# simonhmartin/genomics_general

Measured on AMD Instinct MI355X. Metric: windows_per_sec, higher is better.
Workload: dtype u32 bit-planes / int32 counts / f64 statistics

## Files before the change

### genomics_general_amd/csrc/pg_abi.cpp

```cpp
#include "pg_ctx.h"

#include <sched.h>

#include <algorithm>
#include <chrono>
#include <cstdarg>
#include <cstdio>
#include <cstring>
#include <cstdlib>
#include <thread>

static thread_local char g_err[1024] = "";

int pg_fail(int code, const char *fmt, ...) {
    va_list ap;
    va_start(ap, fmt);
    vsnprintf(g_err, sizeof(g_err), fmt, ap);
    va_end(ap);
    return code;
}

static int usable_cpus() {
    int n = (int)std::thread::hardware_concurrency();
    if (n < 1) n = 1;
// ... 695 lines not shown
        int words = (int)((len + 31) / 32);
        acc += words;
        mw = std::max(mw, words);
        ml = std::max(ml, len);
    }
    h[3 * (size_t)n] = acc;
    if (total_words) *total_words = acc;
    if (max_words) *max_words = mw;
    if (max_len) *max_len = ml;
    rc0 = c->win.upload(h, 3 * (size_t)n + 1, c->stream);
    if (rc0 != PG_OK) return rc0;
    HIPCHK(hipEventRecord(c->win_ev, c->stream));
    return PG_OK;
}

template <class F>
static int pairwise_batches(pg_ctx *c, const int64_t *lo, const int64_t *hi, int n_win, bool dip, F consume) {
    const int N = c->n_hap, NP = c->NP;
    const int n_units = dip ? N / 2 : N;
    const int NPv = dip ? (NP % 64 ? (n_units + 31) / 32 * 32 : (n_units + 63) / 64 * 64) : NP;
    c->cN = n_units;
    c->cshift = dip ? 1 : 0;
    const int64_t mat_bytes = 4ll * N * N + 4ll * n_units * n_units;
    int grp = PG_GROUP;
    {
        int64_t blocks64 = 0;
        for (int w = 0; w < n_win; ++w) blocks64 += ((hi[w] - lo[w] + 31) / 32 + PG_GROUP - 1) / PG_GROUP;
        const int waves_per_block = (NP / 4 + 63) / 64;
        if (blocks64 * waves_per_block >= 32768) grp = PG_GROUP_MAX;
        else if (blocks64 * waves_per_block < 8192) grp = PG_GROUP / 2;
        if (const char *g = getenv("PG_GROUP_WORDS")) grp = std::min(PG_GROUP_MAX, std::max(8, atoi(g) / 4 * 4));
    }
    const int capg = c->xv_worst ? PG_XV_CAP(grp) : PG_XV_CAP_DEFAULT(grp);
    const int64_t word_bytes = ((int64_t)NP * 4 * PG_XV_PLANES * capg + grp - 1) / grp + (int64_t)NPv * 4;
    int64_t total_words_all = 0;
    for (int w = 0; w < n_win; ++w) total_words_all += ((hi[w] - lo[w] + 31) / 32 + grp - 1) / grp * grp;
    const bool multi = total_words_all * word_bytes + (int64_t)n_win * mat_bytes > c->scratch_limit;
    const bool two_streams = getenv("PG_OVERLAP") != nullptr;
    const int n_sub = two_streams && atoi(getenv("PG_OVERLAP")) >= 2 ? atoi(getenv("PG_OVERLAP")) : 8;
    const bool split = multi || two_streams;
    int64_t target_words = two_streams ? std::max<int64_t>(total_words_all / n_sub, 32768) : total_words_all;
    for (int k = 0; k < 2; ++k) {
        if (!c->slot[k].packed) HIPCHK(hipEventCreateWithFlags(&c->slot[k].packed, hipEventDisableTiming));
        if (!c->slot[k].consumed) HIPCHK(hipEventCreateWithFlags(&c->slot[k].consumed, hipEventDisableTiming));
        c->slot[k].used = false;
    }
    int w0 = 0, bi = 0;
    while (w0 < n_win) {
        int64_t words = 0;
        int w1 = w0;
        while (w1 < n_win) {
            int64_t wlen = ((hi[w1] - lo[w1] + 31) / 32 + grp - 1) / grp * grp;
            int64_t nbytes = (words + wlen) * word_bytes + (int64_t)(w1 - w0 + 1) * mat_bytes;
            if (w1 > w0 && (nbytes > (split ? c->scratch_limit / 2 : c->scratch_limit) || words + wlen > target_words)) break;
            words += wlen;
            ++w1;
            if (w1 - w0 >= 65535) break;
        }
        const int nb = w1 - w0;
        pg_ctx::Slot &sl = c->slot[bi & 1];
        int rc;
        const bool single = (w0 == 0 && w1 == n_win) || !two_streams;
        hipStream_t ps = single ? c->stream : c->stream2;
        if (sl.used) {
            HIPCHK(hipStreamWaitEvent(ps, sl.consumed, 0));
            HIPCHK(hipEventSynchronize(sl.packed));
        }
        int64_t ga_pre = 0;
        for (int k = 0; k < nb; ++k) ga_pre += ((hi[w0 + k] - lo[w0 + k] + 31) / 32 + grp - 1) / grp;
        const size_t n_nw = (size_t)nb + (pg_pack_needs_presence(NP) ? (size_t)ga_pre : 0);
        const size_t h_len = 4 * (size_t)nb + 2 + (n_nw + 1) / 2;
        if ((rc = sl.host.ensure(h_len)) != PG_OK) return rc;
        int64_t *h = sl.host.p;
        int64_t ga = 0, va = 0;
        int max_groups = 0;
        for (int k = 0; k < nb; ++k) {
            h[k] = lo[w0 + k];
            h[nb + k] = hi[w0 + k];
            const int64_t wds = (hi[w0 + k] - lo[w0 + k] + 31) / 32;
            h[2 * (size_t)nb + k] = ga;
            h[3 * (size_t)nb + 1 + k] = va;
            const int64_t groups = (wds + grp - 1) / grp;
            ga += groups;
            va += (wds + 3) / 4;
            max_groups = (int)std::max<int64_t>(max_groups, groups);
        }
        h[3 * (size_t)nb] = ga;
        h[4 * (size_t)nb + 1] = va;
        memset(h + 4 * (size_t)nb + 2, 0, ((n_nw + 1) / 2) * 8);
        if ((rc = sl.win.upload(h, h_len, ps)) != PG_OK) return rc;
        const int64_t *d_lo = sl.win.p, *d_hi = sl.win.p + nb, *d_goff = sl.win.p + 2 * (size_t)nb,
                      *d_vgoff = sl.win.p + 3 * (size_t)nb + 1;
        int32_t *d_nw = reinterpret_cast<int32_t *>(sl.win.p + 4 * (size_t)nb + 2);
        if ((rc = sl.Vp.ensure((size_t)(std::max<int64_t>(va, 1) + 4) * NPv * 4)) != PG_OK) return rc;
        if ((rc = sl.XV.ensure(((size_t)std::max<int64_t>(ga, 1) * capg + 4) * PG_XV_PLANES * NP)) != PG_OK) return rc;
        if ((rc = c->Cmat.ensure((size_t)nb * n_units * n_units)) != PG_OK) return rc;
        if ((rc = c->Dmat.ensure((size_t)nb * N * N)) != PG_OK) return rc;
        hipEvent_t e0, e1;
        const bool time_pack = (c->time_mask >> PG_K_PACK) & 1u;
        if (time_pack) {
            if ((rc = event_get(c, &e0)) != PG_OK) return rc;
            if ((rc = event_get(c, &e1)) != PG_OK) return rc;
            HIPCHK(hipEventRecord(e0, ps));
        }
        if (pg_pack_needs_presence(NP) && (rc = sl.pres.ensure((size_t)std::max<int64_t>(ga, 1) * grp * 4)) != PG_OK) return rc;
        pg_launch_pack2(ps, c->gt.p, c->RS, d_lo, d_hi, d_goff, d_vgoff, nb, max_groups, ga, sl.Vp.p, NPv, sl.XV.p, NP,
                        d_nw, dip ? 1 : 0, c->flag.p, sl.pres.p, capg, grp);
        if (time_pack) {
            HIPCHK(hipEventRecord(e1, ps));
            c->events[PG_K_PACK].push_back(std::make_pair(e0, e1));
            c->acc_launches[PG_K_PACK] += 1;
        }
        HIPCHK(hipEventRecord(sl.packed, ps));
        if (!single) HIPCHK(hipStreamWaitEvent(c->stream, sl.packed, 0));
        if ((rc = pg_time_begin(c, PG_K_PAIRWISE, &e0, &e1)) != PG_OK) return rc;
        const bool valu_pairs = getenv("PG_PAIR_VALU") != nullptr;
        if (valu_pairs && NP % 64) return pg_fail(PG_ERR_STATE, "PG_PAIR_VALU must be set before pg_set_samples (plane stride %d)", NP);
        if (!valu_pairs && pg_pair_big_fits(NPv, n_units)) {
            pg_launch_pairC_big(c->stream, sl.Vp.p, d_vgoff, nb, NPv, n_units, dip ? 1 : 0, va / nb, (int64_t)max_groups * grp * 32, c->Cmat.p);
        } else if (!valu_pairs && pg_pair_tile_fits(NPv)) {
            if (pg_launch_pairC_tile(c->stream, sl.Vp.p, d_vgoff, nb, NPv, n_units, dip ? 1 : 0, va / nb, (int64_t)max_groups * grp * 32, c->Cmat.p))
                return pg_fail(PG_ERR_HIP, "pair-kernel program upload failed");
        } else if (!valu_pairs) pg_launch_pairC_mfma(c->stream, sl.Vp.p, d_vgoff, nb, NPv, n_units, dip ? 1 : 0, va / nb, (int64_t)max_groups * grp * 32, c->Cmat.p);
        else if (dip) pg_launch_pairC(c->stream, sl.Vp.p, d_vgoff, nb, c->tasksC.p, c->n_tasksC, NPv, n_units, 1, va / nb, c->Cmat.p);
        else pg_launch_pairC(c->stream, sl.Vp.p, d_vgoff, nb, c->tasksCh.p, c->n_tasksCh, NPv, n_units, 0, va / nb, c->Cmat.p);
        if ((rc = pg_time_end(c, PG_K_PAIRWISE, e0, e1, 1)) != PG_OK) return rc;
        if ((rc = pg_time_begin(c, PG_K_PAIRD, &e0, &e1)) != PG_OK) return rc;
        if (!valu_pairs) pg_launch_pairD_mfma(c->stream, sl.XV.p, d_nw, d_goff, nb, NP, N, ga / nb * grp / 10, (int64_t)max_groups * capg * 32, c->Dmat.p, capg);
        else pg_launch_pairD(c->stream, sl.XV.p, d_nw, d_goff, nb, c->tasks2.p, c->n_tasks2, NP, N, ga / nb, c->Dmat.p, capg);
        if ((rc = pg_time_end(c, PG_K_PAIRD, e0, e1, 1)) != PG_OK) return rc;
        HIPCHK(hipGetLastError());
        c->cur_win_lo = d_lo;
        c->cur_win_hi = d_hi;
        if ((rc = consume(w0, nb)) != PG_OK) return rc;
        HIPCHK(hipEventRecord(sl.consumed, c->stream));
        sl.used = true;
        w0 = w1;
        ++bi;
    }
    for (int k = 0; k < 2; ++k)
        if (c->slot[k].used) HIPCHK(hipEventSynchronize(c->slot[k].packed));
    return PG_OK;
}

static int stream_wait(pg_ctx *c) {
    static const long spin_us = getenv("PG_SPIN_US") ? atol(getenv("PG_SPIN_US")) : 2000;
    if (spin_us > 0) {
        const auto t0 = std::chrono::steady_clock::now();
        for (;;) {
            hipError_t e = hipStreamQuery(c->stream);
            if (e == hipSuccess) return PG_OK;
            if (e != hipErrorNotReady) return pg_fail(PG_ERR_HIP, "hipStreamQuery: %s", hipGetErrorString(e));
            if (std::chrono::duration_cast<std::chrono::microseconds>(std::chrono::steady_clock::now() - t0).count() > spin_us) break;
        }
    }
    HIPCHK(hipStreamSynchronize(c->stream));
    return PG_OK;
}

static int flag_ready(pg_ctx *c) {
    if (c->flag.p) return PG_OK;
    int rc = c->flag.ensure(1);
    if (rc != PG_OK) return rc;
    HIPCHK(hipMemsetAsync(c->flag.p, 0, 4, c->stream));
    HIPCHK(hipStreamSynchronize(c->stream));
    return PG_OK;
}

static int note_flags(pg_ctx *c, int flag, bool *dip, bool *again) {
    *again = false;
    if (flag & PG_FLAG_XV_OVERFLOW) {
        if (c->xv_worst) return pg_fail(PG_ERR_STATE, "XV overflow with the worst-case reservation");
        c->xv_worst = true;
        for (int k = 0; k < 2; ++k) c->slot[k].XV.release();
        *again = true;
    }
    if (*dip && (flag & PG_FLAG_MISMATCH)) {
        *dip = false;
        *again = true;
    }
    return PG_OK;
}

template <class F>
static int pairwise_run(pg_ctx *c, const int64_t *lo, const int64_t *hi, int n_win, F consume) {
    bool dip = c->all_diploid && getenv("PG_NO_DIP") == nullptr;
    int rc;
    if ((rc = flag_ready(c)) != PG_OK) return rc;
    for (;;) {
        if ((rc = pairwise_batches(c, lo, hi, n_win, dip, consume)) != PG_OK) return rc;
        int32_t flag = 0;
        HIPCHK(hipMemcpyAsync(&flag, c->flag.p, 4, hipMemcpyDeviceToHost, c->stream));
        HIPCHK(hipMemsetAsync(c->flag.p, 0, 4, c->stream));
        HIPCHK(hipStreamSynchronize(c->stream));
        bool again;
        if ((rc = note_flags(c, flag, &dip, &again)) != PG_OK) return rc;
        if (!again) return PG_OK;
    }
}

extern "C" int pg_reserve_sites_tuned(pg_ctx *c, int64_t n_sites, int max_trials, double *probe_ms_out, int *n_trials_out,
                                      int *chosen_out) {
    if (!c) return pg_fail(PG_ERR_ARG, "null ctx");
// ... 801 lines not shown
```

### genomics_general_amd/csrc/pg_internal.h

```cpp
#pragma once
#include <hip/hip_runtime.h>
#include <stdint.h>
#include "../../include/popgen_hip.h"
#include "pg_nib.h"

#define PG_MAX_POPS 16
#define PG_SITES_PER_BLOCK 1024
#define PG_ABBA_SITES_PER_BLOCK 4096
#define PG_ABBA_NSUM 6
#define PG_FOURPOP_NSUM 14
#define PG_XV_PLANES 2

#define PG_GROUP 64
#define PG_GROUP_MAX 128
#define PG_XV_CAP(grp) (3 * (grp))
#define PG_XV_CAP_DEFAULT(grp) ((grp) + 1)
#define PG_NP_MAX_SITES 256
#define PG_FLAG_MISMATCH 1
#define PG_FLAG_XV_OVERFLOW 2

struct PgTask2 {
    int32_t row0, nsub, col0, lower;
};

struct PgSynthParams {
    uint64_t seed;
    int64_t first_site_index, scaf_len;
    int32_t n_dip, n_pops, var_thr, miss_thr;
};


void pg_launch_nib_pack(hipStream_t st, const int8_t *src, int S, int n_hap, int64_t n_rows, int8_t *gt, int RS);
void pg_launch_nib_expand(hipStream_t st, const int8_t *gt, int RS, int64_t n_rows, int8_t *dst, int S);
void pg_launch_synth(hipStream_t st, int8_t *gt, int RS, int n_hap, int64_t site0, int64_t n_sites,
                     const int32_t *slot_gen_hap, PgSynthParams p);

void pg_launch_popdist_fin(hipStream_t st, const int32_t *Cmat, const int32_t *Dmat, int N, int cN, int cshift, int n_win,
                           const int32_t *pop_start, int n_pops, int min_pair_sites, double *sum_out,
                           int64_t *cnt_out, int all_diploid, const int64_t *win_lo = nullptr, const int64_t *win_hi = nullptr,
                           long long skip_upto = -1);

void pg_launch_popdist_np(hipStream_t st, const int32_t *Cmat, const int32_t *Dmat, int N, int cN, int cshift, int n_win,
                          const int32_t *pop_start, int n_pops, const int32_t *ref_row, const int32_t *pop_rank,
                          const int32_t *task_tree, const int32_t *trees, int max_leaves, int max_side, int min_pair_sites,
                          double min_data, int do_pairs, double *sums, int64_t *cnts, double *out, const int64_t *win_lo,
                          const int64_t *win_hi, long long max_sites);

void pg_launch_indpair_fin(hipStream_t st, const int32_t *Cmat, const int32_t *Dmat, int N, int cN, int cshift, int n_win,
                           const int32_t *samp_start, const int32_t *samp_rank, int n_samp, int min_pair_sites, double *sum_out,
                           int64_t *cnt_out, int mean_mode);


void pg_launch_abba(hipStream_t st, const int8_t *gt, int RS, const int64_t *win_lo, const int64_t *win_hi,
                    int n_win, int max_chunks, const int32_t *pop_start, int p1, int p2, int p3, int p4,
                    double min_data, int sel, int nsum, double *part_sums, int64_t *part_used, double *sums_out,
                    int64_t *used_out, uint32_t *flags, int64_t base, long long max_sites);

void pg_launch_popfreq(hipStream_t st, const int8_t *gt, int RS, int n_hap, const int64_t *win_lo,
                       const int64_t *win_hi, int n_win, int max_chunks, const int32_t *pop_start, int n_pops,
                       unsigned long long *l_out, unsigned long long *S_out, unsigned long long *pairsum_out,
                       uint32_t *flags, int64_t base);
void pg_launch_popfreq_ordered(hipStream_t st, const int8_t *gt, int RS, const int64_t *win_lo, const int64_t *win_hi, int n_win,
                               const int32_t *pop_start, int n_pops, const uint32_t *flags, int64_t base, double *theta_out);

void pg_launch_site_counts(hipStream_t st, const int8_t *gt, int RS, int64_t site_lo, int64_t site_hi,
                           const int32_t *pop_start, int n_pops, int32_t *cnt_out);
void pg_launch_site_target(hipStream_t st, const int32_t *cnt, int64_t n_sites, int n_pops, int target, double min_data, int as_counts,
                           int has_threshold, double threshold, double *f_out, long long *i_out, uint8_t *keep_out);

void pg_launch_hap_called(hipStream_t st, const int8_t *gt, int RS, int n_hap, const int64_t *win_lo,
                          const int64_t *win_hi, int n_win, int max_chunks, unsigned long long *out);

void pg_launch_pack2(hipStream_t st, const int8_t *gt, int RS, const int64_t *win_lo, const int64_t *win_hi,
                     const int64_t *goff, const int64_t *vgoff, int n_win, int max_groups, int64_t total_groups, uint32_t *Vp,
                     int NPv, uint32_t *XV, int NP, int32_t *nw, int dip, int32_t *mismatch, uint32_t *pres, int capg, int grp);
bool pg_pack_needs_presence(int NP);
void pg_launch_expand(hipStream_t st, const int32_t *Cmat, const int32_t *Dmat, int N, int cN, int cshift, int n_win,
                      int32_t *Cfull, int32_t *Dfull);
void pg_launch_pairC(hipStream_t st, const uint32_t *Vp, const int64_t *vgoff, int n_win, const PgTask2 *tasks, int n_tasks,
                     int NPv, int n_units, int diag, int64_t avg_wq, int32_t *Cmat);
void pg_launch_pairD(hipStream_t st, const uint32_t *XY, const int32_t *nw, const int64_t *goff, int n_win,
                     const PgTask2 *tasks, int n_tasks, int NP, int N, int64_t avg_groups, int32_t *Dmat, int capg);
void pg_launch_pairC_mfma(hipStream_t st, const uint32_t *Vp, const int64_t *vgoff, int n_win, int NPv, int n_units, int diag,
                          int64_t avg_wq, int64_t max_sites, int32_t *Cmat);
void pg_launch_pairD_mfma(hipStream_t st, const uint32_t *XV, const int32_t *nw, const int64_t *goff, int n_win, int NP, int N,
                          int64_t avg_words, int64_t max_vsites, int32_t *Dmat, int capg);

bool pg_pair_tile_fits(int NPv);
int pg_launch_pairC_tile(hipStream_t st, const uint32_t *Vp, const int64_t *vgoff, int n_win, int NPv, int n_units, int diag,
                         int64_t avg_wq, int64_t max_sites, int32_t *Cmat);

bool pg_pair_big_fits(int NPv, int n_units);
void pg_launch_pairC_big(hipStream_t st, const uint32_t *Vp, const int64_t *vgoff, int n_win, int NPv, int n_units, int diag,
                         int64_t avg_wq, int64_t max_sites, int32_t *Cmat);

void pg_launch_sample_het(hipStream_t st, const int32_t *Cmat, const int32_t *Dmat, int N, int cN, int cshift, int n_win,
                          const int32_t *samp_start, int n_samp, int min_pair_sites, double *out);
void pg_launch_hapstats(hipStream_t st, const int32_t *Cmat, const int32_t *Dmat, int N, int cN, int cshift, int n_win,
                        const int32_t *pop_start, int n_pops, int max_pop, const int32_t *order, int min_pair_sites, int diag_nan,
                        double max_dist, uint32_t *bits, size_t bits_per_window, double *out);
void pg_launch_unpack(hipStream_t st, const uint8_t *cells, int n_cols, int64_t n_rows, const int32_t *slot_src, int n_hap,
                      int8_t *gt, int RS);
void pg_launch_flag_export(hipStream_t st, int32_t *flag, double *dst);
void pg_launch_popstats(hipStream_t st, const double *sums, const int64_t *cnts, int n_win, const int32_t *pop_start,
                        int n_pops, double min_data, int do_pairs, double *out, const int64_t *win_lo = nullptr,
                        const int64_t *win_hi = nullptr, long long skip_upto = -1);
```

### genomics_general_amd/csrc/pg_pair2.hip

```cpp
#include "pg_internal.h"

typedef __attribute__((address_space(4))) const uint32_t CU32;

__device__ __forceinline__ void store16(uint32_t *p, uint32_t a, uint32_t b, uint32_t c, uint32_t d) {
    *reinterpret_cast<uint4 *>(p) = make_uint4(a, b, c, d);
}

__device__ __forceinline__ void btrans4(uint32_t t0, uint32_t t1, uint32_t t2, uint32_t t3, uint32_t r[4]) {
    const uint32_t lo01 = __builtin_amdgcn_perm(t1, t0, 0x05010400u), hi01 = __builtin_amdgcn_perm(t1, t0, 0x07030602u);
    const uint32_t lo23 = __builtin_amdgcn_perm(t3, t2, 0x05010400u), hi23 = __builtin_amdgcn_perm(t3, t2, 0x07030602u);
    r[0] = __builtin_amdgcn_perm(lo23, lo01, 0x05040100u);
    r[1] = __builtin_amdgcn_perm(lo23, lo01, 0x07060302u);
    r[2] = __builtin_amdgcn_perm(hi23, hi01, 0x05040100u);
    r[3] = __builtin_amdgcn_perm(hi23, hi01, 0x07060302u);
}

struct RowOff { int v[16]; };

__device__ __forceinline__ RowOff make_row_off(int RS) {
    RowOff ro;
#pragma unroll
    for (int s = 0; s < 16; ++s) {
        int t = s * RS;
        asm volatile("" : "+s"(t));
        ro.v[s] = t;
    }
    return ro;
}

__device__ __forceinline__ void word_load(__amdgpu_buffer_rsrc_t rsrc, int b0, int RS, int row0, const RowOff &ro, uint32_t d[32]) {
    const int v0 = b0 + row0 * RS, v1 = v0 + 16 * RS;
#pragma unroll
    for (int s = 0; s < 16; ++s) d[s] = (uint32_t)__builtin_amdgcn_raw_buffer_load_b32(rsrc, v0, ro.v[s], 0);
// ... 322 lines not shown
    if (cnt) flush();
    if (DIP && bad) atomicOr(mismatch, 1);
}

__device__ __forceinline__ uint32_t bfi_f0(uint32_t hi, uint32_t lo) { return (hi & 0xF0F0F0F0u) | (lo & 0x0F0F0F0Fu); }

__device__ __forceinline__ void word_called_presence_keep(const uint32_t d[32], uint32_t v[8], uint32_t pa[4], uint32_t R[4][8]) {
#pragma unroll
    for (int q = 0; q < 4; ++q) {
        const uint32_t *e = d + 8 * q;
        uint32_t re[4], ro[4];
        btrans4(bfi_f0(e[1] << 4, e[0]), bfi_f0(e[3] << 4, e[2]), bfi_f0(e[5] << 4, e[4]), bfi_f0(e[7] << 4, e[6]), re);
        btrans4(bfi_f0(e[1], e[0] >> 4), bfi_f0(e[3], e[2] >> 4), bfi_f0(e[5], e[4] >> 4), bfi_f0(e[7], e[6] >> 4), ro);
#pragma unroll
        for (int k = 0; k < 4; ++k) {
            R[q][2 * k] = re[k];
            R[q][2 * k + 1] = ro[k];
        }
        const uint32_t o = (re[0] | re[1] | re[2] | re[3]) | (ro[0] | ro[1] | ro[2] | ro[3]);
#pragma unroll
        for (int a = 0; a < 4; ++a) {
            const uint32_t piece = (a >= q ? (o >> (a - q)) : (o << (q - a))) & (0x11111111u << q);
            pa[a] = q ? (pa[a] | piece) : piece;
        }
#pragma unroll
        for (int k = 0; k < 8; ++k) {
            const uint32_t t = R[q][k] + 0x77777777u;
            const uint32_t c = (q == 3 ? t : (t >> (3 - q))) & (0x11111111u << q);
            v[k] = q ? (v[k] | c) : c;
        }
    }
}

constexpr int PACK_CELLS = 24;
template <int TPB, int DIP, int BURST>
__global__ __launch_bounds__(TPB) void k_pack3(const int8_t *__restrict__ gt, int RS, const int64_t *__restrict__ win_lo,
                                               const int64_t *__restrict__ win_hi, const int64_t *__restrict__ goff,
                                               const int64_t *__restrict__ vgoff, uint32_t *__restrict__ Vp, int NPv,
                                               uint32_t *__restrict__ XV, int NP, int32_t *__restrict__ nw,
                                               int32_t *__restrict__ mismatch, int capg, int grp, int fq, int perm) {
    constexpr int NWAVE = TPB / 64;
    constexpr int VN = DIP ? 4 : 8;
    const int FQ = fq, xc = (PACK_CELLS - fq * VN) / 4;
    __shared__ uint32_t sh_pres[2][NWAVE][4];
    __shared__ int sh_slot;
    __shared__ uint4 stage[BURST ? PACK_CELLS * TPB : 1];
    uint4 *const stage_v = stage, *const stage_x = stage + FQ * VN * TPB;
    int nq = 0, nxs = 0, wq_first = 0;
    const int b = (int)(((unsigned long long)blockIdx.y * (unsigned)perm) % gridDim.y), g = blockIdx.x;
    const int64_t lo = win_lo[b], hi = win_hi[b];
    const int W = (int)((hi - lo + 31) >> 5);
    const int w_begin = g * grp;
    if (w_begin >= W) return;
    const int w_end = (w_begin + grp < W) ? w_begin + grp : W;
    const int t = threadIdx.x;
    const int lane = threadIdx.x & 63;
    const int h0 = 8 * t;
    const bool has_data = h0 < 2 * RS;
    const int u0 = DIP ? 4 * t : h0;
    const int64_t first = lo + 32ll * w_begin;
    const int nrows = (int)((hi - first) < 32ll * grp ? (hi - first) : 32ll * grp);
    const __amdgpu_buffer_rsrc_t rsrc = group_rsrc(gt, RS, first, nrows);
    int cnt = 0, parity = 0;
    uint32_t MA = 0u, ME = 0u;
    uint32_t cur[8], xo[8], vo[8];
#pragma unroll
    for (int k = 0; k < 8; ++k) cur[k] = xo[k] = vo[k] = 0u;
    uint32_t bad = 0u;
    uint32_t *xv_base = XV + (size_t)goff[b] * capg * PG_XV_PLANES * (size_t)NP;
    const int capw = (int)(goff[b + 1] - goff[b]) * capg;
    const int64_t vg_base = vgoff[b] + (int64_t)(w_begin >> 2);
    auto reserve = [&](int n) -> int {
        int slot;
// ... 168 lines not shown
            if (has_data) {
#pragma unroll
                for (int k = 0; k < VN; ++k) {
                    const int hk = DIP ? 2 * k : k;
                    stage_v[(nq * VN + k) * TPB + t] = make_uint4(vhold[hk][0], vhold[hk][1], vhold[hk][2], vhold[hk][3]);
                }
            }
            if (++nq == FQ) flush_v();
        } else if (has_data) {
            uint32_t *o = Vp + ((size_t)(vg_base + wq) * NPv + u0) * 4u;
#pragma unroll
            for (int k = 0; k < VN; ++k) {
                const int hk = DIP ? 2 * k : k;
                store16(o + 4 * k, vhold[hk][0], vhold[hk][1], vhold[hk][2], vhold[hk][3]);
            }
        }
    }
    if (cnt & 7) finish_dword(cnt >> 3);
    if (cnt) store_word();
    if (BURST) {
        flush_v();
        flush_x();
    }
    if (DIP && bad) atomicOr(mismatch, 1);
}

template <int DIP>
static void launch_pack2(hipStream_t st, int threads, dim3 grid, const int8_t *gt, int RS, const int64_t *win_lo,
                         const int64_t *win_hi, const int64_t *goff, const int64_t *vgoff, uint32_t *Vp, int NPv, uint32_t *XV,
                         int NP, int32_t *nw, int32_t *mismatch, uint32_t *pres, int capg, int grp) {
    const bool force2 = getenv("PG_PACK2") != nullptr;
    if (threads <= 1024 && !force2) {
        const int lanes = (threads + 1) / 2;
#define PG_PACK3B(T, B) hipLaunchKernelGGL((k_pack3<T, DIP, B>), grid, dim3(T), 0, st, gt, RS, win_lo, win_hi, goff, vgoff, Vp, NPv, XV, NP, nw, mismatch, capg, grp, fq, perm)
#define PG_PACK3(T) PG_PACK3B(T, 0)
        const int fq = DIP ? 4 : 2;
        int perm = 1;
        if (const char *pe = getenv("PG_PACK_PERM")) {
            const int k = atoi(pe), n = (int)grid.y;
            if (k > 1 && n > 2 * k) {
                auto gcd = [](int a, int b) { while (b) { const int t = a % b; a = b; b = t; } return a; };
                perm = n / k;
                while (gcd(perm, n) != 1) ++perm;
            }
        }
        const bool burst = getenv("PG_PACK_BURST") == nullptr || atoi(getenv("PG_PACK_BURST")) != 0;
        if (lanes <= 64 && burst) PG_PACK3B(64, 1);
        else if (lanes <= 128 && burst) PG_PACK3B(128, 1);
        else if (lanes <= 64) PG_PACK3(64);
        else if (lanes <= 128) PG_PACK3(128);
        else if (lanes <= 256) PG_PACK3(256);
        else PG_PACK3(512);
#undef PG_PACK3
#undef PG_PACK3B
        return;
    }
    if (threads <= 64)
        hipLaunchKernelGGL((k_pack2<64, DIP, 0>), grid, dim3(64), 0, st, gt, RS, win_lo, win_hi, goff, vgoff, Vp, NPv, XV, NP, nw, mismatch, pres, capg, grp);
    else if (threads <= 128)
        hipLaunchKernelGGL((k_pack2<128, DIP, 0>), grid, dim3(128), 0, st, gt, RS, win_lo, win_hi, goff, vgoff, Vp, NPv, XV, NP, nw, mismatch, pres, capg, grp);
    else if (threads <= 256)
        hipLaunchKernelGGL((k_pack2<256, DIP, 0>), grid, dim3(256), 0, st, gt, RS, win_lo, win_hi, goff, vgoff, Vp, NPv, XV, NP, nw, mismatch, pres, capg, grp);
    else {
        grid.z = (threads + 255) / 256;
        hipLaunchKernelGGL(k_presence, grid, dim3(256), 0, st, gt, RS, win_lo, win_hi, goff, pres, grp);
        hipLaunchKernelGGL(k_word_scan, dim3(grid.y), dim3(256), 0, st, win_lo, win_hi, goff, pres, nw, grp);
        hipLaunchKernelGGL((k_pack2<256, DIP, 1>), grid, dim3(256), 0, st, gt, RS, win_lo, win_hi, goff, vgoff, Vp, NPv, XV, NP, nw, mismatch, pres, capg, grp);
    }
}

bool pg_pack_needs_presence(int NP) { return NP / 4 > 1024 || (getenv("PG_PACK2") != nullptr && NP / 4 > 256); }

void pg_launch_pack2(hipStream_t st, const int8_t *gt, int RS, const int64_t *win_lo, const int64_t *win_hi,
                     const int64_t *goff, const int64_t *vgoff, int n_win, int max_groups, int64_t total_groups, uint32_t *Vp,
                     int NPv, uint32_t *XV, int NP, int32_t *nw, int dip, int32_t *mismatch, uint32_t *pres, int capg, int grp) {
    if (n_win <= 0 || max_groups <= 0) return;
    const int threads = NP / 4;
    if (pg_pack_needs_presence(NP)) (void)hipMemsetAsync(pres, 0, (size_t)total_groups * grp * 16u, st);
    dim3 grid(max_groups, n_win);
    if (dip) launch_pack2<1>(st, threads, grid, gt, RS, win_lo, win_hi, goff, vgoff, Vp, NPv, XV, NP, nw, mismatch, pres, capg, grp);
    else launch_pack2<0>(st, threads, grid, gt, RS, win_lo, win_hi, goff, vgoff, Vp, NPv, XV, NP, nw, mismatch, pres, capg, grp);
}

struct PairCtx {
    int win, row0, nsub, col0, lower, lane, ks;
};

__device__ __forceinline__ bool pair_decode(const PgTask2 *__restrict__ tasks, int n_tasks, int kso, int n_win, PairCtx &c) {
    const int xcd = blockIdx.x & 7;
    const int v = blockIdx.x >> 3;
    const int per_win = n_tasks * kso;
    const int full = n_win >> 3;
    int rem;
    if (v < full * per_win) {
        c.win = (v / per_win) * 8 + xcd;
        rem = v % per_win;
    } else {
        const int total = (n_win & 7) * per_win, q = (total + 7) >> 3;
        const int vt = v - full * per_win, lin = xcd * q + vt;
        if (vt >= q || lin >= total) return false;
        c.win = full * 8 + lin / per_win;
// ... 192 lines not shown
```

Measured before the change: 323,000.

## Fuse genotype packing with the pairwise-C MFMA product in one kernel

Adds a fused pack kernel where eight waves per block pack genotype words into XV and, in a rotating ring of LDS fragment buffers, accumulate the C pairwise matrix with FP8/FP4 scaled MFMA. It removes the Vp intermediate buffer and the separate pairC kernel launch when there are many windows and more than 128 units. Windows can be split across several blocks, which then combine their results with atomics. The cost is more LDS per block, intra-workgroup spin waits with a stall flag, and lower occupancy.

```diff
diff --git a/genomics_general_amd/csrc/pg_abi.cpp b/genomics_general_amd/csrc/pg_abi.cpp
--- a/genomics_general_amd/csrc/pg_abi.cpp
+++ b/genomics_general_amd/csrc/pg_abi.cpp
@@ -751,7 +751,8 @@
         if (const char *g = getenv("PG_GROUP_WORDS")) grp = std::min(PG_GROUP_MAX, std::max(8, atoi(g) / 4 * 4));
     }
     const int capg = c->xv_worst ? PG_XV_CAP(grp) : PG_XV_CAP_DEFAULT(grp);
-    const int64_t word_bytes = ((int64_t)NP * 4 * PG_XV_PLANES * capg + grp - 1) / grp + (int64_t)NPv * 4;
+    const bool fused = pg_pack_fuse_fits(NP, NPv, n_units, n_win);
+    const int64_t word_bytes = ((int64_t)NP * 4 * PG_XV_PLANES * capg + grp - 1) / grp + (fused ? 0 : (int64_t)NPv * 4);
     int64_t total_words_all = 0;
     for (int w = 0; w < n_win; ++w) total_words_all += ((hi[w] - lo[w] + 31) / 32 + grp - 1) / grp * grp;
     const bool multi = total_words_all * word_bytes + (int64_t)n_win * mat_bytes > c->scratch_limit;
@@ -793,10 +794,13 @@
         int64_t *h = sl.host.p;
         int64_t ga = 0, va = 0;
         int max_groups = 0;
+        int64_t max_wds = 0, sum_wds = 0;
         for (int k = 0; k < nb; ++k) {
             h[k] = lo[w0 + k];
             h[nb + k] = hi[w0 + k];
             const int64_t wds = (hi[w0 + k] - lo[w0 + k] + 31) / 32;
+            max_wds = std::max(max_wds, wds);
+            sum_wds += wds;
             h[2 * (size_t)nb + k] = ga;
             h[3 * (size_t)nb + 1 + k] = va;
             const int64_t groups = (wds + grp - 1) / grp;
@@ -811,7 +815,7 @@
         const int64_t *d_lo = sl.win.p, *d_hi = sl.win.p + nb, *d_goff = sl.win.p + 2 * (size_t)nb,
                       *d_vgoff = sl.win.p + 3 * (size_t)nb + 1;
         int32_t *d_nw = reinterpret_cast<int32_t *>(sl.win.p + 4 * (size_t)nb + 2);
-        if ((rc = sl.Vp.ensure((size_t)(std::max<int64_t>(va, 1) + 4) * NPv * 4)) != PG_OK) return rc;
+        if (!fused && (rc = sl.Vp.ensure((size_t)(std::max<int64_t>(va, 1) + 4) * NPv * 4)) != PG_OK) return rc;
         if ((rc = sl.XV.ensure(((size_t)std::max<int64_t>(ga, 1) * capg + 4) * PG_XV_PLANES * NP)) != PG_OK) return rc;
         if ((rc = c->Cmat.ensure((size_t)nb * n_units * n_units)) != PG_OK) return rc;
         if ((rc = c->Dmat.ensure((size_t)nb * N * N)) != PG_OK) return rc;
@@ -823,8 +827,13 @@
             HIPCHK(hipEventRecord(e0, ps));
         }
         if (pg_pack_needs_presence(NP) && (rc = sl.pres.ensure((size_t)std::max<int64_t>(ga, 1) * grp * 4)) != PG_OK) return rc;
-        pg_launch_pack2(ps, c->gt.p, c->RS, d_lo, d_hi, d_goff, d_vgoff, nb, max_groups, ga, sl.Vp.p, NPv, sl.XV.p, NP,
-                        d_nw, dip ? 1 : 0, c->flag.p, sl.pres.p, capg, grp);
+        if (fused) {
+            if (pg_launch_pack_fused(ps, c->gt.p, c->RS, d_lo, d_hi, d_goff, nb, max_wds, sum_wds / nb, sl.XV.p, NP, d_nw, dip ? 1 : 0,
+                                     c->flag.p, capg, n_units, c->Cmat.p))
+                return pg_fail(PG_ERR_HIP, "the fused pack kernel was refused its LDS");
+        } else
+            pg_launch_pack2(ps, c->gt.p, c->RS, d_lo, d_hi, d_goff, d_vgoff, nb, max_groups, ga, sl.Vp.p, NPv, sl.XV.p, NP,
+                            d_nw, dip ? 1 : 0, c->flag.p, sl.pres.p, capg, grp);
         if (time_pack) {
             HIPCHK(hipEventRecord(e1, ps));
             c->events[PG_K_PACK].push_back(std::make_pair(e0, e1));
@@ -832,10 +841,11 @@
         }
         HIPCHK(hipEventRecord(sl.packed, ps));
         if (!single) HIPCHK(hipStreamWaitEvent(c->stream, sl.packed, 0));
-        if ((rc = pg_time_begin(c, PG_K_PAIRWISE, &e0, &e1)) != PG_OK) return rc;
+        if (!fused && (rc = pg_time_begin(c, PG_K_PAIRWISE, &e0, &e1)) != PG_OK) return rc;
         const bool valu_pairs = getenv("PG_PAIR_VALU") != nullptr;
         if (valu_pairs && NP % 64) return pg_fail(PG_ERR_STATE, "PG_PAIR_VALU must be set before pg_set_samples (plane stride %d)", NP);
-        if (!valu_pairs && pg_pair_big_fits(NPv, n_units)) {
+        if (fused) {
+        } else if (!valu_pairs && pg_pair_big_fits(NPv, n_units)) {
             pg_launch_pairC_big(c->stream, sl.Vp.p, d_vgoff, nb, NPv, n_units, dip ? 1 : 0, va / nb, (int64_t)max_groups * grp * 32, c->Cmat.p);
         } else if (!valu_pairs && pg_pair_tile_fits(NPv)) {
             if (pg_launch_pairC_tile(c->stream, sl.Vp.p, d_vgoff, nb, NPv, n_units, dip ? 1 : 0, va / nb, (int64_t)max_groups * grp * 32, c->Cmat.p))
@@ -843,7 +853,7 @@
         } else if (!valu_pairs) pg_launch_pairC_mfma(c->stream, sl.Vp.p, d_vgoff, nb, NPv, n_units, dip ? 1 : 0, va / nb, (int64_t)max_groups * grp * 32, c->Cmat.p);
         else if (dip) pg_launch_pairC(c->stream, sl.Vp.p, d_vgoff, nb, c->tasksC.p, c->n_tasksC, NPv, n_units, 1, va / nb, c->Cmat.p);
         else pg_launch_pairC(c->stream, sl.Vp.p, d_vgoff, nb, c->tasksCh.p, c->n_tasksCh, NPv, n_units, 0, va / nb, c->Cmat.p);
-        if ((rc = pg_time_end(c, PG_K_PAIRWISE, e0, e1, 1)) != PG_OK) return rc;
+        if (!fused && (rc = pg_time_end(c, PG_K_PAIRWISE, e0, e1, 1)) != PG_OK) return rc;
         if ((rc = pg_time_begin(c, PG_K_PAIRD, &e0, &e1)) != PG_OK) return rc;
         if (!valu_pairs) pg_launch_pairD_mfma(c->stream, sl.XV.p, d_nw, d_goff, nb, NP, N, ga / nb * grp / 10, (int64_t)max_groups * capg * 32, c->Dmat.p, capg);
         else pg_launch_pairD(c->stream, sl.XV.p, d_nw, d_goff, nb, c->tasks2.p, c->n_tasks2, NP, N, ga / nb, c->Dmat.p, capg);
@@ -888,6 +898,7 @@
 
 static int note_flags(pg_ctx *c, int flag, bool *dip, bool *again) {
     *again = false;
+    if (flag & PG_FLAG_FUSE_STALL) return pg_fail(PG_ERR_STATE, "the fused pack kernel's waves lost each other");
     if (flag & PG_FLAG_XV_OVERFLOW) {
         if (c->xv_worst) return pg_fail(PG_ERR_STATE, "XV overflow with the worst-case reservation");
         c->xv_worst = true;
diff --git a/genomics_general_amd/csrc/pg_internal.h b/genomics_general_amd/csrc/pg_internal.h
--- a/genomics_general_amd/csrc/pg_internal.h
+++ b/genomics_general_amd/csrc/pg_internal.h
@@ -18,6 +18,7 @@
 #define PG_NP_MAX_SITES 256
 #define PG_FLAG_MISMATCH 1
 #define PG_FLAG_XV_OVERFLOW 2
+#define PG_FLAG_FUSE_STALL 4
 
 struct PgTask2 {
     int32_t row0, nsub, col0, lower;
@@ -75,6 +76,16 @@
                      const int64_t *goff, const int64_t *vgoff, int n_win, int max_groups, int64_t total_groups, uint32_t *Vp,
                      int NPv, uint32_t *XV, int NP, int32_t *nw, int dip, int32_t *mismatch, uint32_t *pres, int capg, int grp);
 bool pg_pack_needs_presence(int NP);
+struct PgFuseArgs {
+    int32_t n_win, kparts, n_units, T, diag;
+    int32_t *Cmat;
+    signed char a[8][4], b[8][2];
+    unsigned char mask[8];
+};
+bool pg_pack_fuse_fits(int NP, int NPv, int n_units, int n_win);
+int pg_launch_pack_fused(hipStream_t st, const int8_t *gt, int RS, const int64_t *win_lo, const int64_t *win_hi, const int64_t *goff,
+                         int n_win, int64_t max_words, int64_t avg_words, uint32_t *XV, int NP, int32_t *nw, int dip, int32_t *mismatch,
+                         int capg, int n_units, int32_t *Cmat);
 void pg_launch_expand(hipStream_t st, const int32_t *Cmat, const int32_t *Dmat, int N, int cN, int cshift, int n_win,
                       int32_t *Cfull, int32_t *Dfull);
 void pg_launch_pairC(hipStream_t st, const uint32_t *Vp, const int64_t *vgoff, int n_win, const PgTask2 *tasks, int n_tasks,
diff --git a/genomics_general_amd/csrc/pg_pair2.hip b/genomics_general_amd/csrc/pg_pair2.hip
--- a/genomics_general_amd/csrc/pg_pair2.hip
+++ b/genomics_general_amd/csrc/pg_pair2.hip
@@ -1,4 +1,8 @@
 #include "pg_internal.h"
+
+#include <algorithm>
+#include <cstdlib>
+#include <cstring>
 
 typedef __attribute__((address_space(4))) const uint32_t CU32;
 
@@ -387,13 +391,325 @@
     }
 }
 
+constexpr int PACK_FUSE_XC = 2;
+constexpr int PACK_FUSE_NB = 3;
+constexpr int PACK_FUSE_SPINS = 1 << 22;
+typedef int fz_v8i __attribute__((ext_vector_type(8)));
+typedef float fz_v16f __attribute__((ext_vector_type(16)));
+
+__device__ __forceinline__ fz_v16f fz_mfma(const fz_v8i &a, const fz_v8i &b, const fz_v16f &c) {
+    return __builtin_amdgcn_mfma_scale_f32_32x32x64_f8f6f4(a, b, c, 4, 4, 0, 0, 0, 0);
+}
+
+__device__ __forceinline__ bool fuse_win_decode(int per_win, int n_win, int &win, int &rem) {
+    const int xcd = blockIdx.x & 7;
+    const int v = blockIdx.x >> 3;
+    const int full = n_win >> 3;
+    if (v < full * per_win) {
+        win = (v / per_win) * 8 + xcd;
+        rem = v % per_win;
+        return true;
+    }
+    const int total = (n_win & 7) * per_win, q = (total + 7) >> 3;
+    const int vt = v - full * per_win, lin = xcd * q + vt;
+    if (vt >= q || lin >= total) return false;
+    win = full * 8 + lin / per_win;
+    rem = lin % per_win;
+    return true;
+}
+
+template <int DIP>
+__device__ __forceinline__ void pack3_fused(const int8_t *__restrict__ gt, int RS, const int64_t *__restrict__ win_lo,
+                                            const int64_t *__restrict__ win_hi, const int64_t *__restrict__ goff,
+                                            uint32_t *__restrict__ XV, int NP, int32_t *__restrict__ nw,
+                                            int32_t *__restrict__ mismatch, int capg, const PgFuseArgs &fa) {
+    constexpr int VN = DIP ? 4 : 8;
+    extern __shared__ uint4 fz_lds[];
+    int b, kp;
+    if (!fuse_win_decode(fa.kparts, fa.n_win, b, kp)) return;
+    const int UW = 32 * fa.T;
+    const int lane = threadIdx.x & 63, wave = __builtin_amdgcn_readfirstlane(threadIdx.x >> 6);
+    uint4 *const frag = fz_lds;
+    uint4 *const stage_x = fz_lds + PACK_FUSE_NB * 8 * UW + wave * (PACK_FUSE_XC * 4 * 64);
+    int *const ready = reinterpret_cast<int *>(fz_lds + PACK_FUSE_NB * 8 * UW + 8 * (PACK_FUSE_XC * 4 * 64)), *const done = ready + PACK_FUSE_NB;
+    const int64_t lo = win_lo[b], hi = win_hi[b];
+    const int W = (int)((hi - lo + 31) >> 5);
+    const int w_begin = (int)((long long)W * kp / fa.kparts), w_end = (int)((long long)W * (kp + 1) / fa.kparts);
+    const int nit = (w_end - w_begin + 7) >> 3;
+    const int h0 = 8 * lane;
+    const bool has_data = h0 < 2 * RS;
+    const int u0 = VN * lane;
+    int cnt = 0, nxs = 0;
+    uint32_t MA = 0u, ME = 0u;
+    uint32_t cur[8], xo[8], vo[8];
+#pragma unroll
+    for (int k = 0; k < 8; ++k) cur[k] = xo[k] = vo[k] = 0u;
+    uint32_t bad = 0u;
+    uint32_t *xv_base = XV + (size_t)goff[b] * capg * PG_XV_PLANES * (size_t)NP;
+    const int capw = (int)(goff[b + 1] - goff[b]) * capg;
+    auto flush_x = [&]() {
+        if (!nxs) return;
+        int s0 = 0;
+        if (lane == 0) s0 = atomicAdd(&nw[b], nxs);
+        const int slot0 = __builtin_amdgcn_readfirstlane(s0);
+        for (int k = 0; k < nxs; ++k) {
+            if (slot0 + k >= capw) {
+                if (lane == 0) atomicOr(mismatch, 2);
+            } else if (has_data) {
+                uint4 *o = reinterpret_cast<uint4 *>(xv_base + (size_t)(slot0 + k) * PG_XV_PLANES * (size_t)NP + 2 * h0);
+#pragma unroll
+                for (int i = 0; i < 4; ++i) o[i] = stage_x[(4 * k + i) * 64 + lane];
+            }
+        }
+        nxs = 0;
+    };
+    auto store_word = [&]() {
+        if (has_data) {
+#pragma unroll
+            for (int i = 0; i < 4; ++i) stage_x[(4 * nxs + i) * 64 + lane] = make_uint4(xo[2 * i], vo[2 * i], xo[2 * i + 1], vo[2 * i + 1]);
+        }
+        if (++nxs == PACK_FUSE_XC) flush_x();
+#pragma unroll
+        for (int k = 0; k < 8; ++k) xo[k] = vo[k] = 0u;
+    };
+    auto finish_dword = [&](int qd) {
+        const uint32_t nME = ~ME;
+#pragma unroll
+        for (int k = 0; k < 8; ++k) {
+            const uint32_t cx = (((cur[k] & MA) + 0x77777777u) >> 3) & 0x11111111u;
+            const uint32_t cv = (((cur[k] & nME) + 0x77777777u) >> 3) & 0x11111111u;
+            xo[k] |= cx << qd;
+            vo[k] |= cv << qd;
+            cur[k] = 0u;
+        }
+        MA = 0u;
+        ME = 0u;
+    };
+    auto append = [&](const uint32_t (&Rq)[8], int j, uint32_t A, uint32_t E) {
+        const int sh = 4 * (cnt & 7);
+#pragma unroll
+        for (int k = 0; k < 8; ++k) cur[k] |= __builtin_amdgcn_ubfe(Rq[k], 4 * j, 4) << sh;
+        MA |= A << sh;
+        ME |= E << sh;
+        ++cnt;
+        if ((cnt & 7) == 0) {
+            finish_dword((cnt >> 3) - 1);
+            if (cnt == 32) {
+                store_word();
+                cnt = 0;
+            }
+        }
+    };
+    auto word_rsrc = [&](int w) -> __amdgpu_buffer_rsrc_t {
+        const int64_t row = lo + 32ll * w;
+        const int n = w < w_end ? (int)((hi - row) < 32 ? (hi - row) : 32) : 0;
+        return group_rsrc(gt, RS, n ? row : lo, n);
+    };
+    const int r = lane & 31, kb = lane >> 5;
+    int ia[4], ib[2];
+#pragma unroll
+    for (int p = 0; p < 4; ++p) ia[p] = kb * UW + 32 * (int)fa.a[wave][p] + r;
+#pragma unroll
+    for (int p = 0; p < 2; ++p) ib[p] = kb * UW + 32 * (int)fa.b[wave][p] + r;
+    fz_v16f acc[4];
+#pragma unroll
+    for (int p = 0; p < 4; ++p)
+#pragma unroll
+        for (int e = 0; e < 16; ++e) acc[p][e] = 0.0f;
+    auto products_step = [&](const uint4 *fb, int s) {
+        {
+            fz_v8i fa_[4], fb_[2];
+#pragma unroll
+            for (int p = 0; p < 4; ++p) {
+                const uint4 x = fb[2 * s * UW + ia[p]];
+                fa_[p][0] = (int)x.x; fa_[p][1] = (int)x.y; fa_[p][2] = (int)x.z; fa_[p][3] = (int)x.w;
+            }
+#pragma unroll
+            for (int p = 0; p < 2; ++p) {
+                const uint4 x = fb[2 * s * UW + ib[p]];
+                fb_[p][0] = (int)x.x; fb_[p][1] = (int)x.y; fb_[p][2] = (int)x.z; fb_[p][3] = (int)x.w;
+            }
+#pragma unroll
+            for (int p = 0; p < 4; ++p)
+                acc[p] = fz_mfma(fa_[p], fb_[p & 1], acc[p]);
+        }
+    };
+    if (threadIdx.x < 2 * PACK_FUSE_NB) ready[threadIdx.x] = threadIdx.x == 2 * PACK_FUSE_NB - 1 ? -8 : 0;
+    for (int i = threadIdx.x; i < 8 * UW; i += 512) frag[(PACK_FUSE_NB - 1) * 8 * UW + i] = make_uint4(0u, 0u, 0u, 0u);
+    bool stalled = false;
+    auto wait_ge = [&](int *ctr, int target) {
+        for (int spins = 0; __builtin_amdgcn_readfirstlane(__hip_atomic_load(ctr, __ATOMIC_ACQUIRE, __HIP_MEMORY_SCOPE_WORKGROUP)) < target;) {
+            __builtin_amdgcn_s_sleep(1);
+            if (++spins > PACK_FUSE_SPINS) { stalled = true; break; }
+        }
+    };
+    auto arrive = [&](int *ctr) {
+        if (lane == 0) __hip_atomic_fetch_add(ctr, 1, __ATOMIC_RELEASE, __HIP_MEMORY_SCOPE_WORKGROUP);
+    };
+    uint32_t dn[32];
+#pragma unroll
+    for (int s = 0; s < 32; ++s) dn[s] = 0u;
+    const RowOff ro = make_row_off(RS);
+    const int lane_off = has_data ? 4 * lane : 0x40000000;
+    word_load(word_rsrc(w_begin + wave), lane_off, RS, 0, ro, dn);
+    __syncthreads();
+    int slot = 0, round8 = 0, pslot = PACK_FUSE_NB - 1, pround8 = -8;
+    for (int it = 0; it < nit; ++it) {
+        const int w = w_begin + 8 * it + wave;
+        uint32_t pa[4] = {0u, 0u, 0u, 0u};
+        uint32_t R[4][8];
+        const bool live = w < w_end;
+        uint32_t d[32];
+#pragma unroll
+        for (int s = 0; s < 32; ++s) d[s] = dn[s];
+        word_load(word_rsrc(w + 8), lane_off, RS, 0, ro, dn);
+        wait_ge(&ready[pslot], pround8 + 8);
+        const uint4 *fb = frag + pslot * 8 * UW;
+#pragma unroll
+        for (int q = 0; q < 4; ++q) {
+            fz_v8i fa_[4], fb_[2];
+#pragma unroll
+            for (int p = 0; p < 4; ++p) {
+                const uint4 x = fb[2 * q * UW + ia[p]];
+                fa_[p][0] = (int)x.x; fa_[p][1] = (int)x.y; fa_[p][2] = (int)x.z; fa_[p][3] = (int)x.w;
+            }
+#pragma unroll
+            for (int p = 0; p < 2; ++p) {
+                const uint4 x = fb[2 * q * UW + ib[p]];
+                fb_[p][0] = (int)x.x; fb_[p][1] = (int)x.y; fb_[p][2] = (int)x.z; fb_[p][3] = (int)x.w;
+            }
+            const uint32_t *e = d + 8 * q;
+            uint32_t re[4], rq[4];
+            __builtin_amdgcn_sched_barrier(0);
+            btrans4(bfi_f0(e[1] << 4, e[0]), bfi_f0(e[3] << 4, e[2]), bfi_f0(e[5] << 4, e[4]), bfi_f0(e[7] << 4, e[6]), re);
+            asm volatile("" : "+v"(re[0]), "+v"(re[1]), "+v"(re[2]), "+v"(re[3]));
+            __builtin_amdgcn_sched_barrier(0);
+            acc[0] = fz_mfma(fa_[0], fb_[0], acc[0]);
+            __builtin_amdgcn_sched_barrier(0);
+            btrans4(bfi_f0(e[1], e[0] >> 4), bfi_f0(e[3], e[2] >> 4), bfi_f0(e[5], e[4] >> 4), bfi_f0(e[7], e[6] >> 4), rq);
+            asm volatile("" : "+v"(rq[0]), "+v"(rq[1]), "+v"(rq[2]), "+v"(rq[3]));
+            __builtin_amdgcn_sched_barrier(0);
+            acc[1] = fz_mfma(fa_[1], fb_[1], acc[1]);
+            __builtin_amdgcn_sched_barrier(0);
+#pragma unroll
+            for (int k = 0; k < 4; ++k) {
+                R[q][2 * k] = re[k];
+                R[q][2 * k + 1] = rq[k];
+            }
+            const uint32_t o = (re[0] | re[1] | re[2] | re[3]) | (rq[0] | rq[1] | rq[2] | rq[3]);
+#pragma unroll
+            for (int a = 0; a < 4; ++a) {
+                const uint32_t piece = (a >= q ? (o >> (a - q)) : (o << (q - a))) & (0x11111111u << q);
+                pa[a] = q ? (pa[a] | piece) : piece;
+            }
+            asm volatile("" : "+v"(pa[0]), "+v"(pa[1]), "+v"(pa[2]), "+v"(pa[3]));
+            __builtin_amdgcn_sched_barrier(0);
+            acc[2] = fz_mfma(fa_[2], fb_[0], acc[2]);
+            acc[3] = fz_mfma(fa_[3], fb_[1], acc[3]);
+            __builtin_amdgcn_sched_barrier(0);
+        }
+        arrive(&done[pslot]);
+        wait_ge(&done[slot], round8);
+        {
+            uint4 *cell = frag + (slot * 8 + wave) * UW + u0;
+#pragma unroll
+            for (int k = 0; k < VN; ++k) {
+                const int hk = DIP ? 2 * k : k;
+                uint32_t c[4];
+#pragma unroll
+                for (int q = 0; q < 4; ++q) {
+                    const uint32_t t = R[q][hk] + 0x77777777u;
+                    if (DIP) bad |= t ^ (R[q][hk + 1] + 0x77777777u);
+                    c[q] = (t >> 3) & 0x11111111u;
+                }
+                if (u0 + k < UW) cell[k] = make_uint4(c[0], c[1], c[2], c[3]);
+            }
+        }
+        arrive(&ready[slot]);
+        if (live) {
+            uint32_t pr[4];
+#pragma unroll
+            for (int a = 0; a < 4; ++a) pr[a] = pa[a];
+            wave_or4(pr);
+            const uint32_t m0 = poly_mask(pr);
+            if (m0) {
+                const int lb = lane & 31;
+                const uint32_t Pl = __builtin_amdgcn_ubfe(pr[0], lb, 1) | (__builtin_amdgcn_ubfe(pr[1], lb, 1) << 1) |
+                                    (__builtin_amdgcn_ubfe(pr[2], lb, 1) << 2) | (__builtin_amdgcn_ubfe(pr[3], lb, 1) << 3);
+                const uint32_t A0l = Pl & (0u - Pl);
+#pragma unroll
+                for (int q = 0; q < 4; ++q) {
+                    uint32_t mq = m0 & (0x11111111u << q);
+                    while (mq) {
+                        const int bit = __builtin_ctz(mq);
+                        mq &= mq - 1u;
+                        append(R[q], bit >> 2, (uint32_t)__builtin_amdgcn_readlane((int)A0l, bit), 0u);
+                    }
+                }
+                const uint32_t m3 = tri_mask(pr);
+                if (m3) {
+#pragma unroll 1
+                    for (int pass = 1; pass < 3; ++pass) {
+                        uint32_t m = pass == 1 ? m3 : quad_mask(pr);
+                        while (m) {
+                            const int bit = __builtin_ctz(m);
+                            m &= m - 1u;
+                            const uint32_t P = (uint32_t)__builtin_amdgcn_readlane((int)Pl, bit);
+                            const uint32_t A0 = P & (0u - P), P1 = P ^ A0, A1 = P1 & (0u - P1), P2 = P1 ^ A1, A2 = P2 & (0u - P2);
+                            const uint32_t A = pass == 1 ? A1 : A2;
+                            const int q = bit & 3;
+                            if (q == 0) append(R[0], bit >> 2, A, (A - 1u) & P);
+                            else if (q == 1) append(R[1], bit >> 2, A, (A - 1u) & P);
+                            else if (q == 2) append(R[2], bit >> 2, A, (A - 1u) & P);
+                            else append(R[3], bit >> 2, A, (A - 1u) & P);
+                        }
+                    }
+                }
+            }
+        }
+        pslot = slot;
+        pround8 = round8;
+        if (++slot == PACK_FUSE_NB) { slot = 0; round8 += 8; }
+    }
+    wait_ge(&ready[pslot], pround8 + 8);
+#pragma unroll
+    for (int q = 0; q < 4; ++q) products_step(frag + pslot * 8 * UW, q);
+    if (stalled && lane == 0) atomicOr(mismatch, PG_FLAG_FUSE_STALL);
+    if (cnt & 7) finish_dword(cnt >> 3);
+    if (cnt) store_word();
+    flush_x();
+    if (DIP && (bad & 0x88888888u)) atomicOr(mismatch, 1);
+    const int n = fa.n_units, atomic = fa.kparts > 1;
+    int32_t *Cw = fa.Cmat + (size_t)b * n * n;
+#pragma unroll
+    for (int p = 0; p < 4; ++p) {
+        if (!((fa.mask[wave] >> p) & 1)) continue;
+        const int I = fa.a[wave][p], J = fa.b[wave][p & 1];
+        const int col = 32 * J + (lane & 31);
+        if (col >= n) continue;
+#pragma unroll
+        for (int reg = 0; reg < 16; ++reg) {
+            const int row = 32 * I + (reg & 3) + 8 * (reg >> 2) + 4 * (lane >> 5);
+            if (row >= n || row > col || (row == col && !fa.diag)) continue;
+            const int32_t v = (int32_t)(acc[p][reg] * 4.0f);
+            int32_t *dst = &Cw[(size_t)row * n + col];
+            if (atomic) { if (v) atomicAdd(dst, v); }
+            else *dst = v;
+        }
+    }
+}
+
 constexpr int PACK_CELLS = 24;
-template <int TPB, int DIP, int BURST>
+template <int TPB, int DIP, int BURST, int FUSE>
 __global__ __launch_bounds__(TPB) void k_pack3(const int8_t *__restrict__ gt, int RS, const int64_t *__restrict__ win_lo,
                                                const int64_t *__restrict__ win_hi, const int64_t *__restrict__ goff,
                                                const int64_t *__restrict__ vgoff, uint32_t *__restrict__ Vp, int NPv,
                                                uint32_t *__restrict__ XV, int NP, int32_t *__restrict__ nw,
-                                               int32_t *__restrict__ mismatch, int capg, int grp, int fq, int perm) {
+                                               int32_t *__restrict__ mismatch, int capg, int grp, int fq, int perm, PgFuseArgs fa) {
+    if constexpr (FUSE) {
+        pack3_fused<DIP>(gt, RS, win_lo, win_hi, goff, XV, NP, nw, mismatch, capg, fa);
+        return;
+    }
     constexpr int NWAVE = TPB / 64;
     constexpr int VN = DIP ? 4 : 8;
     const int FQ = fq, xc = (PACK_CELLS - fq * VN) / 4;
@@ -628,7 +944,7 @@
     const bool force2 = getenv("PG_PACK2") != nullptr;
     if (threads <= 1024 && !force2) {
         const int lanes = (threads + 1) / 2;
-#define PG_PACK3B(T, B) hipLaunchKernelGGL((k_pack3<T, DIP, B>), grid, dim3(T), 0, st, gt, RS, win_lo, win_hi, goff, vgoff, Vp, NPv, XV, NP, nw, mismatch, capg, grp, fq, perm)
+#define PG_PACK3B(T, B) hipLaunchKernelGGL((k_pack3<T, DIP, B, 0>), grid, dim3(T), 0, st, gt, RS, win_lo, win_hi, goff, vgoff, Vp, NPv, XV, NP, nw, mismatch, capg, grp, fq, perm, PgFuseArgs())
 #define PG_PACK3(T) PG_PACK3B(T, 0)
         const int fq = DIP ? 4 : 2;
         int perm = 1;
@@ -663,6 +979,75 @@
         hipLaunchKernelGGL(k_word_scan, dim3(grid.y), dim3(256), 0, st, win_lo, win_hi, goff, pres, nw, grp);
         hipLaunchKernelGGL((k_pack2<256, DIP, 1>), grid, dim3(256), 0, st, gt, RS, win_lo, win_hi, goff, vgoff, Vp, NPv, XV, NP, nw, mismatch, pres, capg, grp);
     }
+}
+
+bool pg_pack_fuse_fits(int NP, int NPv, int n_units, int n_win) {
+    const char *f = getenv("PG_PACK_FUSE");
+    if (f ? atoi(f) == 0 : (n_win < 1024 || n_units <= 128)) return false;
+    for (const char *e : {"PG_PAIR_VALU", "PG_PACK2", "PG_PACK_BURST", "PG_GROUP_WORDS", "PG_PACK_BLOCKS_PER_CU", "PG_OVERLAP", "PG_PACK_PERM"})
+        if (getenv(e)) return false;
+    return NP <= 512 && n_units >= 1 && pg_pair_big_fits(NPv, n_units);
+}
+
+static void pg_fuse_tasks(int T, PgFuseArgs &fa) {
+    memset(fa.a, 0, sizeof fa.a);
+    memset(fa.b, 0, sizeof fa.b);
+    memset(fa.mask, 0, sizeof fa.mask);
+    const int Tb = T == 7 ? 6 : T;
+    int wv = 0;
+    for (int i = 0; i < Tb; i += 2)
+        for (int j = i; j < Tb; j += 2, ++wv)
+            for (int p = 0; p < 4; ++p) {
+                const int I = i + (p >> 1), J = j + (p & 1);
+                if (I < Tb && J < Tb && I <= J) {
+                    fa.a[wv][p] = (signed char)I;
+                    fa.b[wv][p & 1] = (signed char)J;
+                    fa.mask[wv] |= (unsigned char)(1u << p);
+                }
+            }
+    if (T == 7)
+        for (int i = 0; i < 7; i += 4, ++wv) {
+            fa.b[wv][0] = fa.b[wv][1] = 6;
+            for (int p = 0; p < 4 && i + p < 7; ++p) {
+                fa.a[wv][p] = (signed char)(i + p);
+                fa.mask[wv] |= (unsigned char)(1u << p);
+            }
+        }
+}
+
+int pg_launch_pack_fused(hipStream_t st, const int8_t *gt, int RS, const int64_t *win_lo, const int64_t *win_hi, const int64_t *goff,
+                         int n_win, int64_t max_words, int64_t avg_words, uint32_t *XV, int NP, int32_t *nw, int dip, int32_t *mismatch,
+                         int capg, int n_units, int32_t *Cmat) {
+    if (n_win <= 0) return 0;
+    PgFuseArgs fa;
+    fa.n_win = n_win;
+    fa.n_units = n_units;
+    fa.T = (n_units + 31) / 32;
+    fa.diag = dip ? 1 : 0;
+    fa.Cmat = Cmat;
+    pg_fuse_tasks(fa.T, fa);
+    int64_t kparts = n_win >= 1024 ? 1 : (1024 + n_win - 1) / n_win;
+    kparts = std::min<int64_t>(kparts, std::max<int64_t>(1, avg_words / 64));
+    kparts = std::max<int64_t>(kparts, (max_words * 32 + (1 << 23) - 1) >> 23);
+    fa.kparts = (int)kparts;
+    if (kparts > 1) (void)hipMemsetAsync(Cmat, 0, (size_t)n_win * n_units * n_units * 4, st);
+    const size_t lds = (size_t)(PACK_FUSE_NB * 8 * 32 * fa.T + 8 * PACK_FUSE_XC * 4 * 64 + 2) * sizeof(uint4);
+    const int64_t blocks = (int64_t)((n_win + 7) / 8) * kparts * 8;
+#define PG_PACK3F(D)                                                                                                              \
+    do {                                                                                                                          \
+        static bool ready = false;                                   \
+        if (!ready) {                                                                                                             \
+            if (hipFuncSetAttribute(reinterpret_cast<const void *>(&k_pack3<512, D, 0, 1>), hipFuncAttributeMaxDynamicSharedMemorySize, \
+                                    (PACK_FUSE_NB * 8 * 32 * 7 + 8 * PACK_FUSE_XC * 4 * 64 + 2) * (int)sizeof(uint4)) != hipSuccess) return 1; \
+            ready = true;                                                                                                         \
+        }                                                                                                                         \
+        hipLaunchKernelGGL((k_pack3<512, D, 0, 1>), dim3((unsigned)blocks), dim3(512), lds, st, gt, RS, win_lo, win_hi, goff,         \
+                           (const int64_t *)nullptr, (uint32_t *)nullptr, 0, XV, NP, nw, mismatch, capg, 0, 0, 1, fa);           \
+    } while (0)
+    if (dip) PG_PACK3F(1);
+    else PG_PACK3F(0);
+#undef PG_PACK3F
+    return 0;
 }
 
 bool pg_pack_needs_presence(int NP) { return NP / 4 > 1024 || (getenv("PG_PACK2") != nullptr && NP / 4 > 256); }
```

Result: faster. 350,900 (median of 6 runs) (+8.6%).
